# dongzhuoyao/self-guided-diffusion-models

Measured on AMD Instinct MI355X. Metric: cfg_sampled_images_per_sec_64x64_1000step_ddpm, higher is better.
Workload: dtype f32 as 3xf16 split MFMA products, f32 accumulate; 1 GPU; IN64 unet_fast ch128 cluster-k5000 cond_scale=2 bs=40/GPU (UNet batch 80), 1000-step native DDPM; batch_per_gpu=40, unet_batch=80, precision_mode=f16x3, launch=hipGraph-captured step

## Files before the change

include/sgdm_hip.h:

```cpp
#ifndef SGDM_HIP_H
#define SGDM_HIP_H
#include <stdint.h>

#ifdef __cplusplus
extern "C" {
#endif

#define SGD_ABI_VERSION 24
int sgd_abi_version(void);
const char* sgd_build_id(void);

enum { SGD_MODE_FLAT = 0, SGD_MODE_CONV3 = 1 };
enum { SGD_RS_NONE = 0, SGD_RS_AVGPOOL2 = 1, SGD_RS_UP2 = 2,
       SGD_RS_ZEROUP2 = 3 ,
       SGD_RS_UP2_SUBPIXEL = 4 };
enum { SGD_PRO_NONE = 0, SGD_PRO_AFFINE_NC = 1, SGD_PRO_LN_ROW = 2 };
enum { SGD_PREC_F32 = 0, SGD_PREC_F16X3 = 1, SGD_PREC_BF16X3 = 2, SGD_PREC_F16 = 3, SGD_PREC_BF16 = 4 };

typedef struct sgd_igemm_args {
    const float* x0;
    const float* x1;
    int32_t c0, c1;
    int32_t mode;
    int32_t n, hi, wi;
    int32_t ho, wo;
    int32_t m;
    int32_t rows_per_n;
    int32_t stride;
    int32_t resample;
    int32_t pro;
    int32_t pro_silu;
    const float* pa;
    const float* pb;
    const float* pc;
    const void* w;
    int32_t cin_p, cout_p;
    const float* bias;
    const float* res;
    int32_t res_mode;
    float* y;
    int32_t cout;
    int32_t y_ld;
    int32_t orows_in, orows_out, orow_off;
    int32_t prec;
    float drop_p;
    uint32_t drop_seed;
    float* stats;
    const float* w_scale_inv;
    void* work;
    int64_t work_bytes;
    int32_t grid_cap;
    int32_t tune;
} sgd_igemm_args;
enum {
    SGD_TUNE_BN128 = 1,
    SGD_TUNE_BN256 = 2,
    SGD_TUNE_FLAT2 = 4,
    SGD_TUNE_DEFER = 8,
    SGD_TUNE_PLAIN_SCHEDULE = 16,
    SGD_TUNE_NO_SMALL = 64,
    SGD_TUNE_LN_PACKED = 32,
    SGD_TUNE_WGRAD_GENERIC_NARROW = 256,
// ... 38 lines not shown
    float* scale_inv;
    int32_t cout, cin, ksize, transpose;
    int32_t own_amax, reserved0;
} sgd_pack_job;
int sgd_pack_job_blocks(int32_t cout, int32_t cin, int32_t ksize, int32_t prec, int32_t transpose, int32_t* amax_blocks,
                        int32_t* pack_blocks, int32_t* cin_p, int32_t* cout_p );
int sgd_pack_weights_batched(const sgd_pack_job* jobs, int32_t n_jobs, const int32_t* amax_block_job, const int32_t* amax_first,
                             int32_t n_amax_blocks, const int32_t* pack_block_job, const int32_t* pack_first,
                             int32_t n_pack_blocks, int32_t prec, void* stream);

int sgd_linear_splitk(const float* x, int32_t x_ld, const float* w, const float* bias, int32_t m, int32_t n, int32_t k,
                      float* work, int32_t ksplit, float* y, int32_t y_ld, void* stream);
int sgd_linear_splitk_t(const float* x, int32_t x_ld, const float* w, int32_t w_ld, int32_t m, int32_t n, int32_t k,
                        float* work, int32_t ksplit, float* y, int32_t y_ld, void* stream);

int sgd_chan_stats(const float* x, int32_t n, int32_t hw, int32_t c,
                   float* sums , int32_t c_total, int32_t c_off, void* stream);
int sgd_add_rows_nc(float* x, const float* e, int32_t e_ld, int32_t n, int64_t hw, int32_t c, void* stream);
int sgd_stats_reduce(const float* partial, int32_t n, int32_t parts, int32_t c,
                     float* sums , int32_t c_total, int32_t c_off, void* stream);
int sgd_gn_coef_parts(const float* partial0, int32_t parts0, int32_t c0, const float* partial1, int32_t parts1, int32_t c1,
                      float* sums, const float* gamma, const float* beta, const float* film, int32_t film_ld,
                      int32_t n, int32_t groups, int32_t hw, float eps, float* a, float* b, void* stream);
int sgd_gn_coef(const float* sums, const float* gamma, const float* beta,
                const float* film , int32_t film_ld,
                int32_t n, int32_t c, int32_t groups, int32_t hw, float eps,
                float* a, float* b, void* stream);

int sgd_ln_stats(const float* x, int32_t rows, int32_t c, float eps, float* stats , void* stream);
int sgd_ln_apply(const float* x, const float* gamma, const float* beta, const float* res,
                 int32_t rows, int32_t c, float eps, float* out, void* stream);

int sgd_attention(const float* q, int32_t q_ld, int32_t q_hs,
                  const float* k, const float* v, int32_t kv_ld, int32_t kv_hs,
                  int32_t batch, int32_t heads, int32_t tq, int32_t tk, int32_t d, float scale,
                  float* out, int32_t out_ld,
                  float* lse ,
                  void* stream);
int sgd_attention_split(const float* q, int32_t q_ld, int32_t q_hs,
                        const float* k, const float* v, int32_t kv_ld, int32_t kv_hs,
                        int32_t batch, int32_t heads, int32_t tq, int32_t tk, int32_t d, float scale,
                        float* out, int32_t out_ld, float* lse, void* stream);

int sgd_timestep_embedding(const int64_t* t, const float* freqs, int32_t n_src, int32_t n, int32_t dim,
                           float* out, void* stream);
int sgd_cond_select(const void* cond, int32_t is_i64, const uint8_t* mask, const float* null_row,
// ... 170 lines not shown
```

self-guided-diffusion-models_amd/csrc/backward.hip:

```cpp
#include "sgdm_common.h"
#include "../../include/sgdm_hip.h"
#include "prologue.h"

namespace {

__device__ __forceinline__ float dsilu(float z) {
    const float s = 1.0f / (1.0f + __expf(-z));
    return s * (1.0f + z * (1.0f - s));
}

constexpr int WK = 64;
constexpr int WT = 128;
constexpr int WLD = WT + 4;

struct WArgs {
    sgd_igemm_args a;
    const float* gy;
    int gy_ld, cout, ksplit, taps, rows, co_tiles, ci_tiles, ktiles, hc, wc, wo_l2, ho_l2, gvec;
    float* slabs;
    float* bslab;
    const void* gh; const void* gl; const void* uh; const void* ul;
    int no_flat_pipe;
    int tap9;
};
// ... 1611 lines not shown
static bool wgrad_ws_ok(const sgd_igemm_args& a, int cout, int gy_ld) {
    const bool vec = (a.c0 % 4 == 0) && (a.c1 % 4 == 0);
    const bool pooled = a.resample == SGD_RS_AVGPOOL2 && !(a.tune & SGD_TUNE_WGRAD_NO_POOLED_PLANES);
    return wgrad_fast_conv(a) && a.prec != SGD_PREC_F32 && !(a.tune & SGD_TUNE_WGRAD_F32) && vec && gy_ld % 4 == 0 && cout % WT == 0
           && (a.resample == SGD_RS_NONE || a.resample == SGD_RS_UP2 || pooled)
           && (a.pro == SGD_PRO_NONE || a.pro == SGD_PRO_AFFINE_NC) && !(a.tune & SGD_TUNE_WGRAD_NO_WS);
}
static int64_t wgrad_planes_need(const sgd_igemm_args& a, int cout) {
    const int64_t rows = (int64_t)a.n * a.ho * a.wo;
    return 4 * (rows * cout + (int64_t)a.n * a.hi * a.wi * (a.c0 + a.c1));
}
static bool wgrad_planes_ok(const sgd_igemm_args& a, int cout, int gy_ld, bool have_scratch, int64_t scratch_bytes) {
    if (!(wgrad_ws_ok(a, cout, gy_ld) && have_scratch && scratch_bytes >= wgrad_planes_need(a, cout) && !(a.tune & SGD_TUNE_WGRAD_NO_PLANES)))
        return false;
    const long cin = a.c0 + a.c1;
    return cin * cout > 100 * (cin + cout) || a.resample == SGD_RS_AVGPOOL2 || (a.tune & SGD_TUNE_WGRAD_PLANES_ALWAYS);
}

static int wgrad_impl(const sgd_igemm_args* fwd, const float* gy, int32_t gy_ld, int32_t cout, float* slabs,
                      int32_t ksplit, float* bias_slabs, void* scratch, int64_t scratch_bytes, void* stream) {
    SGD_CLEAR_ERR();
    if (!fwd || !gy || !slabs || cout <= 0 || ksplit <= 0 || gy_ld < cout) return SGD_ERR_ARG;
    if (fwd->prec < SGD_PREC_F32 || fwd->prec > SGD_PREC_BF16X3) return SGD_ERR_ARG;
    WArgs w;
    w.a = *fwd;
    w.no_flat_pipe = (fwd->tune & SGD_TUNE_WGRAD_NO_PIPE) ? 1 : 0;
    w.tap9 = 0;
    const sgd_igemm_args& a = w.a;
    if (!a.x0 || a.c0 <= 0 || a.c1 < 0 || (a.c1 > 0 && !a.x1)) return SGD_ERR_ARG;
    if (a.pro != SGD_PRO_NONE && (!a.pa || !a.pb)) return SGD_ERR_ARG;
    const int cin = a.c0 + a.c1;
    if (a.mode == SGD_MODE_CONV3) {
        if (a.stride != 1 && a.stride != 2) return SGD_ERR_ARG;
        w.hc = a.resample == SGD_RS_AVGPOOL2 ? a.hi / 2 : (a.resample == SGD_RS_UP2 ? a.hi * 2 : a.hi);
        w.wc = a.resample == SGD_RS_AVGPOOL2 ? a.wi / 2 : (a.resample == SGD_RS_UP2 ? a.wi * 2 : a.wi);
        w.taps = 9;
        w.rows = a.n * a.ho * a.wo;
        if (a.ho <= 0 || a.wo <= 0 || (a.ho & (a.ho - 1)) || (a.wo & (a.wo - 1))) return SGD_ERR_ARG;
        w.wo_l2 = __builtin_ctz(a.wo);
        w.ho_l2 = __builtin_ctz(a.ho);
    } else if (a.mode == SGD_MODE_FLAT) {
        w.hc = w.wc = 1;
        w.wo_l2 = w.ho_l2 = 0;
        w.taps = 1;
        w.rows = a.m;
    } else {
// ... 271 lines not shown
```

self-guided-diffusion-models_amd/csrc/igemm.hip:

```cpp
#include <type_traits>
#include <utility>

#include "igemm_shared.h"
#include "prologue.h"

namespace {

#ifdef SGDM_PROBE
#define DBG(bit) 0
#define SYNC() do { if (g.stamp) { const unsigned long long t0_ = __builtin_amdgcn_s_memtime(); __syncthreads(); \
                    const unsigned long long t1_ = __builtin_amdgcn_s_memtime(); \
                    if (g.trace && blockIdx.x < 16 && pr_nbar < 512 && (threadIdx.x & 63) == 0) { \
                        unsigned long long* tp_ = g.trace + (((size_t)blockIdx.x * (NTHREADS / 64) + (threadIdx.x >> 6)) * 512 + pr_nbar) * 2; \
                        tp_[0] = t0_; tp_[1] = t1_; } \
                    pr_bar += t1_ - t0_; ++pr_nbar; } else if (!DBG(64)) { __syncthreads(); } } while (0)
#define PROBE_BEGIN() unsigned long long pr_bar = 0, pr_nbar = 0, pr_epi = 0; const unsigned long long pr_t0 = __builtin_amdgcn_s_memtime()
#define PROBE_END(role) do { if (g.stamp && (threadIdx.x & 63) == 0) { \
        unsigned long long* sp_ = g.stamp + ((size_t)blockIdx.x * (NTHREADS / 64) + (threadIdx.x >> 6)) * 4; \
        sp_[0] = __builtin_amdgcn_s_memtime() - pr_t0; sp_[1] = pr_bar; sp_[2] = pr_nbar; sp_[3] = pr_epi; } } while (0)
#define PROBE_EPI(expr) do { if (g.stamp) { const unsigned long long t0_ = __builtin_amdgcn_s_memtime(); expr; pr_epi += __builtin_amdgcn_s_memtime() - t0_; } else { expr; } } while (0)
#else
#define DBG(bit) 0
#define SYNC() __syncthreads()
#define PROBE_BEGIN()
// ... 318 lines not shown

        Q = (ntiles - 1) * nchunks + (last_c1 - last_c0);
        S = Q * TAPS;
        s = CONV ? a.stride : 1;
        TW = 1 << g.tw_l2; TH = 1 << g.th_l2;
        M = CONV ? a.n * a.ho * a.wo : a.m;

        return true;
    }

    __device__ __forceinline__ void build_pixtab(int k, int t0, int nthr) const {
        if (k >= ntiles) return;
        const Tile T = tile_at<SUBPIX>(g, lin_of(k), BN, TW, TH);
        int2* tab = pixtab + (size_t)(k & 3) * g.pix;
        for (int pix = t0; pix < g.pix; pix += nthr) {
            int2 e;
            e.x = -1;
            e.y = 0;
            if (CONV) {
                int hx = pix % g.hw, t = pix / g.hw;
                int hy = t % g.hh, nb = t / g.hh;
                int n = T.img0 + nb, y = T.ty0 * s - 1 + hy, x = T.tx0 * s - 1 + hx;
                if (n < a.n && y >= 0 && y < g.hc && x >= 0 && x < g.wc) {
                    if (a.resample == SGD_RS_UP2) e.x = (n * a.hi + (y >> 1)) * a.wi + (x >> 1);
                    else if (a.resample == SGD_RS_AVGPOOL2) e.x = (n * a.hi + 2 * y) * a.wi + 2 * x;
                    else if (a.resample == SGD_RS_ZEROUP2) e.x = ((y | x) & 1) ? -1 : (n * a.hi + (y >> 1)) * a.wi + (x >> 1);
                    else e.x = (n * a.hi + y) * a.wi + x;
                    e.y = n;
                }
            } else {
                long row = T.m0 + pix;
                if (row < M) {
                    e.x = (int)row;
                    e.y = (a.pro == SGD_PRO_AFFINE_NC) ? (int)(row / a.rows_per_n) : 0;
                }
            }
            tab[pix] = e;
        }
    }

    static constexpr size_t SLAB = (size_t)RB * CBN * QPB * NCOMP * 16;
    static __device__ __forceinline__ f32x4 accq(const AccV (&acc)[RB][CBN], int mt, int nt, int q) {
        f32x4 v;
#pragma unroll
        for (int j = 0; j < 4; ++j) v[j] = acc[mt][nt][(M16 ? 0 : q * 4) + j];
        return v;
    }
    __device__ __forceinline__ int pixel_of_lane(int ln) const {
    const int l5 = ln & 31;
        int px = l5;
// ... 1104 lines not shown
```

self-guided-diffusion-models_amd/csrc/igemm_host.hip:

```cpp
#include <stdint.h>

#include "igemm_shared.h"

extern "C" int sgd_abi_version(void) { return SGD_ABI_VERSION; }

static inline int pick_bn(int cout) { return (cout % 128 == 0) ? 128 : 32; }

static inline int column_tile(const sgd_igemm_args& a) {
    const int bn = pick_bn(a.cout);
    if (bn != 128 || (a.tune & (SGD_TUNE_NO_SMALL | SGD_TUNE_BN128 | SGD_TUNE_BN256))) return bn;
    const long rows = a.mode == SGD_MODE_CONV3 ? (long)a.n * a.ho * a.wo : (long)a.m;
    const long t128 = ((rows + BM - 1) / BM) * ((a.cout + 127) / 128);
    return t128 * 4 <= device_cus() ? 32 : 128;
}

static int make_geo(const sgd_igemm_args& a, Geo& g, int bn, int& na, int fg = 1) {
    if (a.c0 <= 0 || a.c1 < 0 || a.cout <= 0 || a.y_ld < a.cout) return SGD_ERR_ARG;
    if (a.mode == SGD_MODE_CONV3) {
        if (a.n <= 0 || a.hi <= 0 || a.wi <= 0 || (a.stride != 1 && a.stride != 2)) return SGD_ERR_ARG;
        if (a.stride == 2 && a.resample != SGD_RS_NONE) return SGD_ERR_ARG;
        if (a.resample < SGD_RS_NONE || a.resample > SGD_RS_UP2_SUBPIXEL) return SGD_ERR_ARG;
        const bool sub = a.resample == SGD_RS_UP2_SUBPIXEL;
        const bool up = a.resample == SGD_RS_UP2 || a.resample == SGD_RS_ZEROUP2;
        g.hc = a.resample == SGD_RS_AVGPOOL2 ? a.hi / 2 : (up ? a.hi * 2 : a.hi);
// ... 105 lines not shown
    Geo g;
    int na;
    if (make_geo(a, g, 128, na) != SGD_OK) return false;
    if (a.stats && g.sparts == 0) return false;
    const size_t smem = (size_t)na * g.pix * LDA * sizeof(float) + (size_t)g.pix * 32
                        + (a.cout <= BIAS_LDS_MAX ? (size_t)((a.cout + 127) / 128 * 128) * sizeof(float) : 0);
    return smem <= 160 * 1024;
}

extern "C" int sgd_igemm_subpixel_ok(const sgd_igemm_args* args) { return args && subpixel_ok(*args) ? 1 : 0; }

extern "C" int sgd_igemm(const sgd_igemm_args* args, void* stream) {
    SGD_CLEAR_ERR();
    if (!args) return SGD_ERR_ARG;
    KArgs ka;
    ka.a = *args;
    sgd_igemm_args& a = ka.a;
    Geo& g = ka.g;
    if (!a.x0 || !a.w || !a.y || a.c0 <= 0 || a.c1 < 0 || a.cout <= 0) return SGD_ERR_ARG;
    if (a.prec < SGD_PREC_F32 || a.prec > SGD_PREC_BF16) return SGD_ERR_ARG;
    if (a.c1 > 0 && (!a.x1 || a.c0 % KC != 0)) return SGD_ERR_ARG;
    if (a.y_ld < a.cout) return SGD_ERR_ARG;
    if (a.pro != SGD_PRO_NONE && (!a.pa || !a.pb)) return SGD_ERR_ARG;
    const int cin = a.c0 + a.c1;
    int bn = column_tile(a);
    if (a.cout_p % pick_bn(a.cout) != 0 || a.cout_p < a.cout || a.cin_p % KC != 0 || a.cin_p < cin) return SGD_ERR_ARG;
    const bool vec = (a.c0 % 4 == 0) && (a.c1 % 4 == 0);
    const bool conv = a.mode == SGD_MODE_CONV3;
    const bool sub = conv && a.resample == SGD_RS_UP2_SUBPIXEL;
    if (sub && !subpixel_ok(a)) return SGD_ERR_ARG;
    if (bn == 128 && a.cout_p % 256 == 0 && vec && (!a.res || a.res_mode == SGD_RS_NONE) && want_bn256(a)) bn = 256;
    int na;
    int taps = conv ? (sub ? 4 : 9) : 1;
    const bool ln_nopk = !conv && a.pro == SGD_PRO_LN_ROW && a.prec != SGD_PREC_F32 && !(a.tune & SGD_TUNE_LN_PACKED);
    const bool ln_any = !conv && a.pro == SGD_PRO_LN_ROW && (ln_nopk || (a.tune & SGD_TUNE_LN_PACKED));
    if (!conv && vec && bn >= 128 && a.drop_p == 0.f && cin % (2 * KC) == 0 && (a.c1 == 0 || a.c0 % KC == 0)
        && (a.pro == SGD_PRO_NONE || (a.pro == SGD_PRO_AFFINE_NC && a.rows_per_n > 0 && a.rows_per_n % BM == 0) || ln_any)
        && (a.tune & SGD_TUNE_FLAT2))
        taps = 2;
    {
        const int rc = make_geo(a, g, bn, na, conv ? 1 : taps);
        if (rc != SGD_OK) return rc;
    }
    if (a.stats && g.sparts == 0) return SGD_ERR_ARG;
    g.nt = a.cout_p / bn;
    if ((a.work && a.work_bytes < sgd_igemm_work_bytes()) || (a.tune & SGD_TUNE_PLAIN_SCHEDULE)) a.work = nullptr;
// ... 47 lines not shown
```

self-guided-diffusion-models_amd/csrc/norm.hip:

```cpp
#include "sgdm_common.h"
#include "../../include/sgdm_hip.h"

namespace {

__global__ __launch_bounds__(256) void chan_stats_kernel(const float* __restrict__ x, int hw, int c,
                                                         float* __restrict__ sums, int c_total, int c_off) {
    const int slabs = (c + 31) / 32;
    const int n = blockIdx.x / slabs, slab = blockIdx.x % slabs;
    const int q = threadIdx.x & 7, rl = threadIdx.x >> 3;
    const int ch = slab * 32 + q * 4;
    float s[4] = {0, 0, 0, 0}, ss[4] = {0, 0, 0, 0};
    const float* base = x + (long)n * hw * c;
    if (ch < c) {
        if ((c & 3) == 0) {
            for (int r = rl; r < hw; r += 32) {
                f32x4 v = *reinterpret_cast<const f32x4*>(base + (long)r * c + ch);
#pragma unroll
                for (int j = 0; j < 4; ++j) { s[j] += v[j]; ss[j] += v[j] * v[j]; }
            }
        } else {
            for (int r = rl; r < hw; r += 32)
#pragma unroll
                for (int j = 0; j < 4; ++j)
                    if (ch + j < c) { float v = base[(long)r * c + ch + j]; s[j] += v; ss[j] += v * v; }
// ... 46 lines not shown
    for (int k = 0; k < cpg; ++k) {
        s += sums[((long)nn * c + g0 + k) * 2];
        ss += sums[((long)nn * c + g0 + k) * 2 + 1];
    }
    const double cnt = (double)cpg * hw;
    const double mean = s / cnt;
    double var = ss / cnt - mean * mean;
    if (var < 0) var = 0;
    const double rstd = 1.0 / sqrt(var + (double)eps);
    double ga = gamma[cc] * rstd, be = beta[cc] - mean * ga;
    if (film) {
        const double sc = 1.0 + film[(long)nn * film_ld + cc], sh = film[(long)nn * film_ld + c + cc];
        ga *= sc;
        be = be * sc + sh;
    }
    a[i] = (float)ga;
    b[i] = (float)be;
}

__global__ __launch_bounds__(512) void gn_coef_parts_kernel(const float* __restrict__ p0, int parts0, int c0,
                                                            const float* __restrict__ p1, int parts1, int c1,
                                                            float* __restrict__ sums, const float* __restrict__ gamma,
                                                            const float* __restrict__ beta, const float* __restrict__ film,
                                                            int film_ld, int groups, int hw, float eps,
                                                            float* __restrict__ a, float* __restrict__ b) {
    extern __shared__ double shd[];
    const int nn = blockIdx.x, c = c0 + c1, nthr = blockDim.x;
    const int G = c < nthr ? nthr / c : 1;
    float* sh = reinterpret_cast<float*>(shd + (size_t)G * c * 2);
    for (int it = threadIdx.x; it < c * G; it += nthr) {
        const int ch = it % c, grp = it / c;
        const bool first = ch < c0;
        const float* p = first ? p0 : p1;
        const int parts = first ? parts0 : parts1, cs = first ? c0 : c1, cl = first ? ch : ch - c0;
        double t0 = 0, t1 = 0;
        if (parts > 0) {
            const float* q = p + (long)nn * parts * 2 * cs + cl;
            int k = grp;
            for (; k + 7 * G < parts; k += 8 * G) {
                float v0[8], v1[8];
#pragma unroll
                for (int j = 0; j < 8; ++j) { v0[j] = q[(long)(k + j * G) * 2 * cs]; v1[j] = q[(long)(k + j * G) * 2 * cs + cs]; }
#pragma unroll
                for (int j = 0; j < 8; ++j) { t0 += v0[j]; t1 += v1[j]; }
            }
            if (k + 3 * G < parts) {
                float v0[4], v1[4];
#pragma unroll
                for (int j = 0; j < 4; ++j) { v0[j] = q[(long)(k + j * G) * 2 * cs]; v1[j] = q[(long)(k + j * G) * 2 * cs + cs]; }
#pragma unroll
                for (int j = 0; j < 4; ++j) { t0 += v0[j]; t1 += v1[j]; }
                k += 4 * G;
            }
            for (; k < parts; k += G) { t0 += q[(long)k * 2 * cs]; t1 += q[(long)k * 2 * cs + cs]; }
        }
        shd[((size_t)grp * c + ch) * 2] = t0;
        shd[((size_t)grp * c + ch) * 2 + 1] = t1;
    }
    __syncthreads();
    for (int ch = threadIdx.x; ch < c; ch += nthr) {
// ... 164 lines not shown

extern "C" int sgd_stats_reduce(const float* partial, int32_t n, int32_t parts, int32_t c, float* sums,
                                int32_t c_total, int32_t c_off, void* stream) {
    SGD_CLEAR_ERR();
    if (!partial || !sums || n <= 0 || parts <= 0 || c <= 0 || c_off < 0 || c_off + c > c_total) return SGD_ERR_ARG;
    hipLaunchKernelGGL(stats_reduce_kernel, dim3((2 * c + 31) / 32, n), dim3(256), 0, (hipStream_t)stream, partial,
                       parts, c, sums, c_total, c_off);
    return sgd_check_launch();
}

extern "C" int sgd_gn_coef(const float* sums, const float* gamma, const float* beta, const float* film,
                           int32_t film_ld, int32_t n, int32_t c, int32_t groups, int32_t hw, float eps, float* a,
                           float* b, void* stream) {
    SGD_CLEAR_ERR();
    if (!sums || !gamma || !beta || !a || !b || n <= 0 || c <= 0 || groups <= 0 || c % groups != 0 || hw <= 0)
        return SGD_ERR_ARG;
    if (film && film_ld < 2 * c) return SGD_ERR_ARG;
    const long total = (long)n * c;
    hipLaunchKernelGGL(gn_coef_kernel, dim3((unsigned)((total + 255) / 256)), dim3(256), 0, (hipStream_t)stream,
                       sums, gamma, beta, film, film_ld, n, c, groups, hw, eps, a, b);
    return sgd_check_launch();
}

extern "C" int sgd_gn_coef_parts(const float* p0, int32_t parts0, int32_t c0, const float* p1, int32_t parts1, int32_t c1,
                                 float* sums, const float* gamma, const float* beta, const float* film, int32_t film_ld,
                                 int32_t n, int32_t groups, int32_t hw, float eps, float* a, float* b, void* stream) {
    SGD_CLEAR_ERR();
    const int c = c0 + c1;
    if (!sums || !gamma || !beta || !a || !b || n <= 0 || c0 <= 0 || c1 < 0 || groups <= 0 || c % groups != 0 || hw <= 0 ||
        parts0 < 0 || parts1 < 0 || (parts0 > 0 && !p0) || (c1 > 0 && parts1 > 0 && !p1) || c > 8192)
        return SGD_ERR_ARG;
    if (film && film_ld < 2 * c) return SGD_ERR_ARG;
    const int nthr = 512, G = c < nthr ? nthr / c : 1;
    const size_t lds = (size_t)G * c * 2 * sizeof(double) + (size_t)c * 2 * sizeof(float);
    if (lds > 160 * 1024) return SGD_ERR_ARG;
    if (lds > 64 * 1024) {
        static bool raised = false;
        if (!raised) {
            (void)hipFuncSetAttribute((const void*)gn_coef_parts_kernel, hipFuncAttributeMaxDynamicSharedMemorySize, 160 * 1024);
            raised = true;
        }
    }
    hipLaunchKernelGGL(gn_coef_parts_kernel, dim3(n), dim3(nthr), lds,
                       (hipStream_t)stream, p0, parts0, c0, p1, parts1, c1, sums, gamma, beta, film, film_ld, groups, hw, eps, a, b);
    return sgd_check_launch();
}

extern "C" int sgd_ln_stats(const float* x, int32_t rows, int32_t c, float eps, float* stats, void* stream) {
    SGD_CLEAR_ERR();
    if (!x || !stats || rows <= 0 || c <= 0 || c > 1024) return SGD_ERR_ARG;
    hipLaunchKernelGGL((ln_kernel<false>), dim3((rows + 3) / 4), dim3(256), 0, (hipStream_t)stream, x,
                       (const float*)nullptr, (const float*)nullptr, (const float*)nullptr, rows, c, eps, stats);
    return sgd_check_launch();
}

extern "C" int sgd_ln_apply(const float* x, const float* gamma, const float* beta, const float* res, int32_t rows,
                            int32_t c, float eps, float* out, void* stream) {
    SGD_CLEAR_ERR();
    if (!x || !gamma || !out || rows <= 0 || c <= 0 || c > 1024) return SGD_ERR_ARG;
    hipLaunchKernelGGL((ln_kernel<true>), dim3((rows + 3) / 4), dim3(256), 0, (hipStream_t)stream, x, gamma, beta,
                       res, rows, c, eps, out);
    return sgd_check_launch();
}

extern "C" int sgd_ln_bwd(const float* x, const float* g, const float* gamma, int32_t rows, int32_t c, float eps,
                          float* dst, int32_t accumulate, float* gxhat, const float* gres, void* stream) {
    SGD_CLEAR_ERR();
    if (!x || !g || !gamma || !dst || rows <= 0 || c <= 0 || c > 1024) return SGD_ERR_ARG;
// ... 5 lines not shown
```

self-guided-diffusion-models_amd/sgdm_amd/_lib.py:

```python
import ctypes as C
import os

import torch

_HERE = os.path.dirname(os.path.abspath(__file__))
LIB_PATH = os.environ.get("SGDM_LIB_PATH") or os.path.join(_HERE, "lib", "libsgdm_hip.so")

MODE_FLAT, MODE_CONV3 = 0, 1
RS_NONE, RS_AVGPOOL2, RS_UP2, RS_ZEROUP2, RS_UP2_SUBPIXEL = 0, 1, 2, 3, 4
PRO_NONE, PRO_AFFINE_NC, PRO_LN_ROW = 0, 1, 2
PREC_F32, PREC_F16X3, PREC_BF16X3, PREC_F16, PREC_BF16 = 0, 1, 2, 3, 4
PREC_BY_NAME = {"f32": PREC_F32, "f16x3": PREC_F16X3, "bf16x3": PREC_BF16X3, "f16": PREC_F16, "bf16": PREC_BF16}
INFERENCE_ONLY = ("f16", "bf16")
ABI_VERSION = 24

TUNE_BN128, TUNE_BN256, TUNE_FLAT2, TUNE_DEFER, TUNE_PLAIN_SCHEDULE, TUNE_LN_PACKED, TUNE_NO_SMALL = 1, 2, 4, 8, 16, 32, 64
TUNE_WGRAD_GENERIC_NARROW, TUNE_WGRAD_NO_POOLED_PLANES, TUNE_WGRAD_F32 = 256, 512, 1024
TUNE_WGRAD_NO_WS, TUNE_WGRAD_NO_PLANES, TUNE_WGRAD_NO_PIPE, TUNE_WGRAD_PLANES_ALWAYS = 2048, 4096, 8192, 16384
TUNE_NO_SUBPIXEL = 32768
PACK_FORWARD, PACK_DGRAD, PACK_SUBPIXEL = 0, 1, 2

vp, i32, i64, f32 = C.c_void_p, C.c_int32, C.c_int64, C.c_float


class IgemmArgs(C.Structure):
    _fields_ = [
        ("x0", vp), ("x1", vp), ("c0", i32), ("c1", i32), ("mode", i32),
        ("n", i32), ("hi", i32), ("wi", i32), ("ho", i32), ("wo", i32), ("m", i32),
        ("rows_per_n", i32), ("stride", i32), ("resample", i32), ("pro", i32), ("pro_silu", i32),
        ("pa", vp), ("pb", vp), ("pc", vp), ("w", vp), ("cin_p", i32), ("cout_p", i32),
        ("bias", vp), ("res", vp), ("res_mode", i32), ("y", vp), ("cout", i32), ("y_ld", i32),
        ("orows_in", i32), ("orows_out", i32), ("orow_off", i32), ("prec", i32),
        ("drop_p", f32), ("drop_seed", C.c_uint32), ("stats", vp), ("w_scale_inv", vp),
        ("work", vp), ("work_bytes", i64), ("grid_cap", i32), ("tune", i32),
    ]


class PackJob(C.Structure):
    _fields_ = [("src", vp), ("dst", vp), ("amax_bits", vp), ("scale_inv", vp), ("cout", i32), ("cin", i32), ("ksize", i32),
                ("transpose", i32), ("own_amax", i32), ("reserved0", i32)]


SIGNATURES = {
    "sgd_abi_version": (i32, []),
    "sgd_build_id": (C.c_char_p, []),
    "sgd_igemm": (i32, [C.POINTER(IgemmArgs), vp]),
    "sgd_igemm_stats_parts": (i32, [C.POINTER(IgemmArgs)]),
    "sgd_igemm_subpixel_ok": (i32, [C.POINTER(IgemmArgs)]),
    "sgd_igemm_work_bytes": (i64, []),
    "sgd_igemm_work_status_offset": (i64, []),
    "sgd_igemm_tail_layout": (i32, [i32, i32, i32, i32, C.POINTER(i32)]),
    "sgd_stats_reduce": (i32, [vp, i32, i32, i32, vp, i32, i32, vp]),
    "sgd_packed_weight_bytes": (i64, [i32, i32, i32, i32]),
    "sgd_pack_weight": (i32, [vp, vp, i32, i32, i32, i32, C.POINTER(i32), C.POINTER(i32), vp]),
    "sgd_weight_amax": (i32, [vp, i64, vp, vp]),
    "sgd_pack_weight_scaled": (i32, [vp, vp, i32, i32, i32, i32, i32, vp, vp, C.POINTER(i32), C.POINTER(i32), vp]),
    "sgd_packed_weight_subpixel_bytes": (i64, [i32, i32, i32]),
    "sgd_weight_amax_subpixel": (i32, [vp, i32, i32, vp, vp]),
    "sgd_pack_weight_subpixel_scaled": (i32, [vp, vp, i32, i32, i32, vp, vp, C.POINTER(i32), C.POINTER(i32), vp]),
    "sgd_pack_job_blocks": (i32, [i32, i32, i32, i32, i32, C.POINTER(i32), C.POINTER(i32), C.POINTER(i32), C.POINTER(i32)]),
    "sgd_pack_weights_batched": (i32, [vp, i32, vp, vp, i32, vp, vp, i32, i32, vp]),
    "sgd_linear_splitk": (i32, [vp, i32, vp, vp, i32, i32, i32, vp, i32, vp, i32, vp]),
    "sgd_linear_splitk_t": (i32, [vp, i32, vp, i32, i32, i32, i32, vp, i32, vp, i32, vp]),
    "sgd_conv3_narrow_in_parts": (i32, [i32, i32]),
    "sgd_conv3_narrow_in": (i32, [vp, vp, vp, vp, vp, i32, i32, i32, i32, i32, i32, i32, vp]),
    "sgd_conv3_narrow_out": (i32, [vp, vp, vp, i32, vp, vp, vp, i32, i32, i32, i32, i32, i32, vp]),
    "sgd_chan_stats": (i32, [vp, i32, i32, i32, vp, i32, i32, vp]),
    "sgd_gn_coef_parts": (i32, [vp, i32, i32, vp, i32, i32, vp, vp, vp, vp, i32, i32, i32, i32, f32, vp, vp, vp]),
    "sgd_gn_coef": (i32, [vp, vp, vp, vp, i32, i32, i32, i32, i32, f32, vp, vp, vp]),
    "sgd_add_rows_nc": (i32, [vp, vp, i32, i32, i64, i32, vp]),
    "sgd_ln_stats": (i32, [vp, i32, i32, f32, vp, vp]),
    "sgd_ln_apply": (i32, [vp, vp, vp, vp, i32, i32, f32, vp, vp]),
    "sgd_attention": (i32, [vp, i32, i32, vp, vp, i32, i32, i32, i32, i32, i32, i32, f32, vp, i32, vp, vp]),
    "sgd_attention_split": (i32, [vp, i32, i32, vp, vp, i32, i32, i32, i32, i32, i32, i32, f32, vp, i32, vp, vp]),
    "sgd_attention_masked": (i32, [vp, i32, i32, vp, vp, i32, i32, vp, i32, i32, i32, i32, i32, f32, vp, i32, vp, vp]),
    "sgd_linear_attention": (i32, [vp, i32, i32, vp, vp, i32, i32, vp, i32, i32, i32, i32, i32, f32, vp, i32, vp]),
    "sgd_attention_bwd": (i32, [vp, i32, i32, vp, vp, i32, i32, vp, i32, vp, i32, vp, vp, i32, i32, i32, i32, i32, f32,
                              vp, vp, vp, vp]),
    "sgd_attention_bwd_split": (i32, [vp, i32, i32, vp, vp, i32, i32, vp, i32, vp, i32, vp, vp, i32, i32, i32, i32, i32, f32,
                                    vp, vp, vp, vp]),
    "sgd_attention_masked_bwd": (i32, [vp, i32, i32, vp, vp, i32, i32, vp, vp, i32, vp, i32, vp, vp, i32, i32, i32, i32, i32,
                                     f32, vp, vp, vp, vp]),
    "sgd_linear_attention_bwd": (i32, [vp, i32, i32, vp, vp, i32, i32, vp, vp, i32, i32, i32, i32, i32, i32, f32, vp, vp, vp,
                                     vp]),
    "sgd_pack_weight_dgrad": (i32, [vp, vp, i32, i32, i32, i32, C.POINTER(i32), C.POINTER(i32), vp]),
    "sgd_wgrad": (i32, [C.POINTER(IgemmArgs), vp, i32, i32, vp, i32, vp, vp]),
    "sgd_wgrad_scratch_bytes": (i64, [C.POINTER(IgemmArgs), i32]),
    "sgd_wgrad_scratch": (i32, [C.POINTER(IgemmArgs), vp, i32, i32, vp, i32, vp, vp, i64, vp]),
    "sgd_colsum_fold": (i32, [vp, i32, i32, vp, i32, f32, vp]),
    "sgd_wgrad_reduce": (i32, [vp, i32, i32, i32, i32, vp, i32, f32, vp]),
    "sgd_wgrad_reduce_bias": (i32, [vp, i32, i32, i32, i32, vp, i32, f32, vp, i32, vp, vp]),
# ... 104 lines not shown
```

self-guided-diffusion-models_amd/sgdm_amd/unet.py:

```python
import ctypes as C
import weakref
import math
import os

import torch
import torch.nn as nn

from . import _lib as L

GN_GROUPS, GN_EPS, LN_EPS = 32, 1e-5, 1e-5
NUM_TIME_TOKENS = NUM_COND_TOKENS = 8


def _ptr(t):
    return C.c_void_p(t.data_ptr()) if t is not None else C.c_void_p(0)


def timestep_freqs(dim, max_period=10000):
    half = dim // 2
    return torch.exp(-math.log(max_period) * torch.arange(start=0, end=half, dtype=torch.float32) / half)


def default_precision():
    return os.environ.get("SGDM_PREC", "f32")
# ... 487 lines not shown


def grad_health(dev):
    dev = torch.device(dev)
    key = (dev.type, dev.index if dev.index is not None else (torch.cuda.current_device() if dev.type == "cuda" else 0))
    if key not in _GRAD_HEALTH:
        _GRAD_HEALTH[key] = torch.zeros(1, dtype=torch.float32, device=dev)
    return _GRAD_HEALTH[key]


class _Engine:

    def __init__(self, model, n, h, w, prec, dev):
        self.m, self.n, self.h, self.w, self.prec, self.dev = model, n, h, w, prec, dev
        self.lib = L.load()
        self.prog = _Program()
        self.packed = []
        self.bufs = []
        self.tape = []
        self.drops = []
        self.lse = {}
        self.stats_of = {}
        self._p_drop = 0.0
        self._grid_cap = 0
        self.refresh_hooks = []
        self.work_bytes = int(self.lib.sgd_igemm_work_bytes()) if os.environ.get("SGDM_BALANCE", "1") != "0" else 0
        self.work = torch.zeros(max(1, self.work_bytes // 4), dtype=torch.float32, device=dev)
        self._build()

    def buf(self, *shape, dtype=torch.float32):
        t = torch.empty(*shape, dtype=dtype, device=self.dev)
        self.bufs.append(t)
        return t

    def attention_fn(self):
        return self.lib.sgd_attention_split if self.prec in (L.PREC_F16X3, L.PREC_F16) else self.lib.sgd_attention

    def pack(self, names, ksize, pad=None, subpixel=False):
        pk = _Packed([self.m.P(nm) for nm in names], ksize, self.prec, pad, subpixel)
        self.packed.append(pk)
        return pk

    def up_conv(self, tag, x0, c0, y, cout, wname, conv, *, stats=False, **kw):
        assert conv[6] == L.RS_UP2
        pk = self.pack([wname], 3)
        q = L.IgemmArgs()
# ... 98 lines not shown
                return fn(x_p, pa_p, pb_p, int(silu), w_p, b_p, y_p, nimg, ho, wo, c0, cout, y_ld, stream)
            self.prog.add(tag, sgd_conv3_narrow_out, flops=flops, nbytes=nbytes)
        elif launch:
            self.prog.add(tag, self.lib.sgd_igemm, C.byref(a), flops=flops, nbytes=nbytes)
        return a

    def gn(self, tag, srcs, hw, gname, film=None, film_ld=0, eps=GN_EPS):
        n = self.n
        ct = sum(c for _, c in srcs)
        sums = self.buf(n, ct, 2)
        off = 0
        parts = []
        for t, c in srcs:
            st = self.stats_of.get(t.data_ptr())
            if st is not None and st[2] == c:
                parts.append((st[0], st[1], c))
            else:
                self.prog.add(tag + ".stats", self.lib.sgd_chan_stats, _ptr(t), n, hw, c, _ptr(sums), ct, off)
                parts.append((None, 0, c))
            off += c
        a, b = self.buf(n, ct), self.buf(n, ct)
        self._last_sums = sums
        gw, gb = self.m.P(gname + ".weight"), self.m.P(gname + ".bias")
        if len(parts) <= 2 and any(p[1] > 0 for p in parts):
            (p0, n0, c0), (p1, n1, c1) = parts[0], (parts[1] if len(parts) == 2 else (None, 0, 0))
            self.prog.add(tag + ".coef", self.lib.sgd_gn_coef_parts, _ptr(p0) if p0 is not None else None, n0, c0,
                          _ptr(p1) if p1 is not None else None, n1, c1, _ptr(sums), _ptr(gw), _ptr(gb),
                          C.c_void_p(film or 0), film_ld, n, GN_GROUPS, hw, eps, _ptr(a), _ptr(b))
        else:
            self.prog.add(tag + ".coef", self.lib.sgd_gn_coef, _ptr(sums), _ptr(gw), _ptr(gb), C.c_void_p(film or 0),
                          film_ld, n, ct, GN_GROUPS, hw, eps, _ptr(a), _ptr(b))
        return a, b

    def _build(self):
        m, n, H, W = self.m, self.n, self.h, self.w
        self._late = []
        mc = m.model_channels
        ted = 4 * mc
        P = m.P
        lib = self.lib
        self.temb = self.buf(n, mc)
        self.freqs = timestep_freqs(mc).to(self.dev)
        cin_tot = m._in_ch_total
        self.x_in = self.buf(n, H, W, cin_tot)
        self.cond_m = self.buf(n, max(1, m._cond_width)) if m._cond_width else None
        emb = self.buf(n, ted)
        e1 = self.buf(n, ted)
        a0 = self.igemm("time_embed.0", self.temb, mc, e1, ted, self.pack(["time_embed.0.weight"], 1), m=n,
                        bias=P("time_embed.0.bias"))
        a2 = self.igemm("time_embed.2", e1, ted, emb, ted, self.pack(["time_embed.2.weight"], 1), m=n, silu=1,
                        bias=P("time_embed.2.bias"))
        self.tape.append(dict(kind="mlp2", name="time_embed", x=self.temb, h=e1, y=emb, a0=a0, a2=a2, cin=mc,
                              mid=ted, cout=ted, add_to_y=False))
        self.context = None
        self.emb_c = None
# ... 57 lines not shown
                               stats=True)
                self.tape.append(dict(kind="down", p=p, x=t, y=y, c=c, hw_in=(hh, ww), a=a))
                srcs = [(y, c, hh // 2, ww // 2)]
            elif kind == "up":
                (t, c, hh, ww), = srcs
                y = self.buf(self.n, hh * 2, ww * 2, c)
                a = self.up_conv(p + ".conv", t, c, y, c, p + ".conv.weight",
                                 (self.n, hh, ww, hh * 2, ww * 2, 1, L.RS_UP2), bias=self.m.P(p + ".conv.bias"), stats=True)
                self.tape.append(dict(kind="up", p=p, x=t, y=y, c=c, hw_in=(hh, ww), a=a))
                srcs = [(y, c, hh * 2, ww * 2)]
        return srcs[0]

    def _res(self, p, layer, srcs):
        _, cin, cout, ud = layer
        n, P = self.n, self.m.P
        t0, c0, hh, ww = srcs[0]
        t1, c1 = (srcs[1][0], srcs[1][1]) if len(srcs) == 2 else (None, 0)
        assert c0 + c1 == cin
        rs = {None: L.RS_NONE, "down": L.RS_AVGPOOL2, "up": L.RS_UP2}[ud]
        ho, wo = (hh // 2, ww // 2) if ud == "down" else ((hh * 2, ww * 2) if ud == "up" else (hh, ww))
        ss = self.m.use_scale_shift_norm
        a1, b1 = self.gn(p + ".in_layers.0", [(t0, c0)] + ([(t1, c1)] if t1 is not None else []), hh * ww,
                         p + ".in_layers.0")
        sums1 = self._last_sums
        h1 = self.buf(n, ho, wo, cout)
        kw1 = dict(x1=t1, c1=c1, pro=L.PRO_AFFINE_NC, silu=1, pa=a1, pb=b1, bias=P(p + ".in_layers.2.bias"), stats=ss)
        if rs == L.RS_UP2:
            ac1 = self.up_conv(p + ".in_layers.2", t0, c0, h1, cout, p + ".in_layers.2.weight", (n, hh, ww, ho, wo, 1, rs), **kw1)
        else:
            ac1 = self.igemm(p + ".in_layers.2", t0, c0, h1, cout, self.pack([p + ".in_layers.2.weight"], 3),
                             conv=(n, hh, ww, ho, wo, 1, rs), **kw1)
        film_ptr = self.film.data_ptr() + 4 * self.film_off[p]
        if ss:
            a2, b2 = self.gn(p + ".out_layers.0", [(h1, cout)], ho * wo, p + ".out_layers.0", film=film_ptr,
                             film_ld=self.film_ld)
        else:
            self.prog.add(p + ".emb_add", self.lib.sgd_add_rows_nc, _ptr(h1), C.c_void_p(film_ptr), self.film_ld, n, ho * wo, cout)
            a2, b2 = self.gn(p + ".out_layers.0", [(h1, cout)], ho * wo, p + ".out_layers.0")
        sums2 = self._last_sums
        ask = None
        if cin != cout:
            assert ud is None
            skip = self.buf(n, hh, ww, cout)
            ask = self.igemm(p + ".skip_connection", t0, c0, skip, cout,
                             self.pack([p + ".skip_connection.weight"], 1), x1=t1, c1=c1, m=n * hh * ww,
                             bias=P(p + ".skip_connection.bias"))
            res, res_mode = skip, L.RS_NONE
        else:
            assert t1 is None
            res, res_mode = t0, rs
        y = self.buf(n, ho, wo, cout)
        ac2 = self.igemm(p + ".out_layers.3", h1, cout, y, cout, self.pack([p + ".out_layers.3.weight"], 3),
                         conv=(n, ho, wo, ho, wo, 1, L.RS_NONE), pro=L.PRO_AFFINE_NC, silu=1, pa=a2, pb=b2,
                         bias=P(p + ".out_layers.3.bias"), res=res, res_mode=res_mode, stats=True)
        pbox, sbox = C.c_float(0.0), C.c_uint32(0)
        self.drops.append((ac2, pbox, sbox))
        self.tape.append(dict(kind="res", drop_p=pbox, drop_seed=sbox, p=p,
                              srcs=[(t0, c0)] + ([(t1, c1)] if t1 is not None else []), cin=cin,
                              cout=cout, hw_in=(hh, ww), hw_out=(ho, wo), rs=rs, a1=a1, b1=b1, sums1=sums1, h1=h1,
                              a2=a2, b2=b2, sums2=sums2, film_off=self.film_off[p], conv1=ac1, conv2=ac2, skip=ask,
                              y=y, ss=ss))
        return (y, cout, ho, wo)

    def refresh(self, stream):
        if getattr(self, "_pack_batch", None) is None or len(self._pack_batch.packs) != len(self.packed):
            self._pack_batch = _PackBatch(self.packed, self.prec, self.dev)
        self._pack_batch.refresh(stream)
        for a, pk in self._late:
            a.cin_p, a.cout_p = pk.cin_p, pk.cout_p
        for hook in self.refresh_hooks:
            hook(stream)
        sig = tuple((b.data_ptr(), b._version) for b in self._film_bias_src)
        if sig != getattr(self, "_film_sig", None):
            self._film_bias.copy_(torch.cat([b.detach().reshape(-1) for b in self._film_bias_src]))
            self._film_sig = sig

    def _health_fail(self, training=False):
        self.work.zero_()
        what = ("sgdm_amd: a conv launch's balanced tail timed out waiting for another block's partial sums (stale arrival "
# ... 47 lines not shown
            bw.apply_grid_cap()

    def run(self, x, t, cond, layout, mask, train=False):
        stream = torch.cuda.current_stream().cuda_stream
        self.prepare(x, t, cond, layout, mask, train=train)
        self.launch(stream)

    def prepare(self, x, t, cond, layout, mask, train=False):
        m, n = self.m, self.n
        stream = torch.cuda.current_stream().cuda_stream
        self.poll_health()
        self.refresh(stream)
        from .ddp import reserved_cus
        self.set_grid_cap(reserved_cus(m) if train else 0)
        p_drop = float(m.dropout) if (train and m.dropout) else 0.0
        if p_drop != self._p_drop or p_drop > 0:
            seeds = torch.randint(0, 2 ** 31 - 1, (len(self.drops),)).tolist() if p_drop > 0 else [0] * len(self.drops)
            for (a, pbox, sbox), sd in zip(self.drops, seeds):
                a.drop_p, a.drop_seed = p_drop, sd
                pbox.value, sbox.value = p_drop, sd
            self._p_drop = p_drop
        B = x.shape[0]
        assert n % B == 0
        x = x.contiguous().float()
        t = t.contiguous().to(torch.int64)
        mask_u8 = mask.contiguous().view(torch.uint8) if mask is not None else None
        cl = m._in_ch_total - m.in_channels
        lfmt = 0
        if cl:
            if layout is None:
                raise ValueError(f"condition_method={m.condition_method} needs `layout`")
            if layout.dtype == torch.uint8 and layout.numel() == B * self.h * self.w:
                layout, lfmt = layout.contiguous(), 1
            elif layout.dtype in (torch.int32, torch.int64) and tuple(layout.shape) == (B, 4):
                if cl != 1:
                    raise ValueError("box-corner layouts need layout_dim == 1")
                layout, lfmt = layout.to(torch.int32).contiguous(), 2
            else:
                layout = layout.contiguous().float()
                assert layout.shape == (B, cl, self.h, self.w), (layout.shape, (B, cl, self.h, self.w))
        is_i64 = 0
        if m._cond_width:
            if cond is None:
                raise ValueError(f"condition_method={m.condition_method} needs `cond`")
            cond = cond.contiguous()
            if cond.dtype == torch.int64 and cond.numel() == B and m._cond_width > 1:
# ... 532 lines not shown
```

Baseline: 2.325 images/s.

## Share first resblock conv and GN stats between CFG cond/uncond halves

```diff
diff --git a/include/sgdm_hip.h b/include/sgdm_hip.h
--- a/include/sgdm_hip.h
+++ b/include/sgdm_hip.h
@@ -38,6 +38,7 @@
     const float* bias;
     const float* res;
     int32_t res_mode;
+    int32_t x_imgs;
     float* y;
     int32_t cout;
     int32_t y_ld;
@@ -122,6 +123,9 @@
 int sgd_gn_coef_parts(const float* partial0, int32_t parts0, int32_t c0, const float* partial1, int32_t parts1, int32_t c1,
                       float* sums, const float* gamma, const float* beta, const float* film, int32_t film_ld,
                       int32_t n, int32_t groups, int32_t hw, float eps, float* a, float* b, void* stream);
+int sgd_gn_coef_parts_shared(const float* partial0, int32_t parts0, int32_t c0, const float* partial1, int32_t parts1, int32_t c1,
+                             float* sums, const float* gamma, const float* beta, const float* film, int32_t film_ld,
+                             int32_t n, int32_t stats_imgs, int32_t groups, int32_t hw, float eps, float* a, float* b, void* stream);
 int sgd_gn_coef(const float* sums, const float* gamma, const float* beta,
                 const float* film , int32_t film_ld,
                 int32_t n, int32_t c, int32_t groups, int32_t hw, float eps,
diff --git a/self-guided-diffusion-models_amd/csrc/backward.hip b/self-guided-diffusion-models_amd/csrc/backward.hip
--- a/self-guided-diffusion-models_amd/csrc/backward.hip
+++ b/self-guided-diffusion-models_amd/csrc/backward.hip
@@ -1657,6 +1657,7 @@
     SGD_CLEAR_ERR();
     if (!fwd || !gy || !slabs || cout <= 0 || ksplit <= 0 || gy_ld < cout) return SGD_ERR_ARG;
     if (fwd->prec < SGD_PREC_F32 || fwd->prec > SGD_PREC_BF16X3) return SGD_ERR_ARG;
+    if (fwd->x_imgs != 0) return SGD_ERR_ARG;
     WArgs w;
     w.a = *fwd;
     w.no_flat_pipe = (fwd->tune & SGD_TUNE_WGRAD_NO_PIPE) ? 1 : 0;
diff --git a/self-guided-diffusion-models_amd/csrc/igemm.hip b/self-guided-diffusion-models_amd/csrc/igemm.hip
--- a/self-guided-diffusion-models_amd/csrc/igemm.hip
+++ b/self-guided-diffusion-models_amd/csrc/igemm.hip
@@ -364,10 +364,11 @@
                 int hy = t % g.hh, nb = t / g.hh;
                 int n = T.img0 + nb, y = T.ty0 * s - 1 + hy, x = T.tx0 * s - 1 + hx;
                 if (n < a.n && y >= 0 && y < g.hc && x >= 0 && x < g.wc) {
-                    if (a.resample == SGD_RS_UP2) e.x = (n * a.hi + (y >> 1)) * a.wi + (x >> 1);
-                    else if (a.resample == SGD_RS_AVGPOOL2) e.x = (n * a.hi + 2 * y) * a.wi + 2 * x;
-                    else if (a.resample == SGD_RS_ZEROUP2) e.x = ((y | x) & 1) ? -1 : (n * a.hi + (y >> 1)) * a.wi + (x >> 1);
-                    else e.x = (n * a.hi + y) * a.wi + x;
+                    const int ns = a.x_imgs > 0 ? n % a.x_imgs : n;
+                    if (a.resample == SGD_RS_UP2) e.x = (ns * a.hi + (y >> 1)) * a.wi + (x >> 1);
+                    else if (a.resample == SGD_RS_AVGPOOL2) e.x = (ns * a.hi + 2 * y) * a.wi + 2 * x;
+                    else if (a.resample == SGD_RS_ZEROUP2) e.x = ((y | x) & 1) ? -1 : (ns * a.hi + (y >> 1)) * a.wi + (x >> 1);
+                    else e.x = (ns * a.hi + y) * a.wi + x;
                     e.y = n;
                 }
             } else {
diff --git a/self-guided-diffusion-models_amd/csrc/igemm_host.hip b/self-guided-diffusion-models_amd/csrc/igemm_host.hip
--- a/self-guided-diffusion-models_amd/csrc/igemm_host.hip
+++ b/self-guided-diffusion-models_amd/csrc/igemm_host.hip
@@ -151,6 +151,7 @@
     if (a.c1 > 0 && (!a.x1 || a.c0 % KC != 0)) return SGD_ERR_ARG;
     if (a.y_ld < a.cout) return SGD_ERR_ARG;
     if (a.pro != SGD_PRO_NONE && (!a.pa || !a.pb)) return SGD_ERR_ARG;
+    if (a.x_imgs < 0 || (a.x_imgs > 0 && (a.mode != SGD_MODE_CONV3 || a.drop_p != 0.f))) return SGD_ERR_ARG;
     const int cin = a.c0 + a.c1;
     int bn = column_tile(a);
     if (a.cout_p % pick_bn(a.cout) != 0 || a.cout_p < a.cout || a.cin_p % KC != 0 || a.cin_p < cin) return SGD_ERR_ARG;
diff --git a/self-guided-diffusion-models_amd/csrc/norm.hip b/self-guided-diffusion-models_amd/csrc/norm.hip
--- a/self-guided-diffusion-models_amd/csrc/norm.hip
+++ b/self-guided-diffusion-models_amd/csrc/norm.hip
@@ -92,10 +92,11 @@
                                                             const float* __restrict__ p1, int parts1, int c1,
                                                             float* __restrict__ sums, const float* __restrict__ gamma,
                                                             const float* __restrict__ beta, const float* __restrict__ film,
-                                                            int film_ld, int groups, int hw, float eps,
+                                                            int film_ld, int stats_imgs, int groups, int hw, float eps,
                                                             float* __restrict__ a, float* __restrict__ b) {
     extern __shared__ double shd[];
     const int nn = blockIdx.x, c = c0 + c1, nthr = blockDim.x;
+    const int ns = stats_imgs > 0 ? nn % stats_imgs : nn;
     const int G = c < nthr ? nthr / c : 1;
     float* sh = reinterpret_cast<float*>(shd + (size_t)G * c * 2);
     for (int it = threadIdx.x; it < c * G; it += nthr) {
@@ -105,7 +106,7 @@
         const int parts = first ? parts0 : parts1, cs = first ? c0 : c1, cl = first ? ch : ch - c0;
         double t0 = 0, t1 = 0;
         if (parts > 0) {
-            const float* q = p + (long)nn * parts * 2 * cs + cl;
+            const float* q = p + (long)ns * parts * 2 * cs + cl;
             int k = grp;
             for (; k + 7 * G < parts; k += 8 * G) {
                 float v0[8], v1[8];
@@ -316,11 +317,13 @@
     return sgd_check_launch();
 }
 
-extern "C" int sgd_gn_coef_parts(const float* p0, int32_t parts0, int32_t c0, const float* p1, int32_t parts1, int32_t c1,
-                                 float* sums, const float* gamma, const float* beta, const float* film, int32_t film_ld,
-                                 int32_t n, int32_t groups, int32_t hw, float eps, float* a, float* b, void* stream) {
+extern "C" int sgd_gn_coef_parts_shared(const float* p0, int32_t parts0, int32_t c0, const float* p1, int32_t parts1, int32_t c1,
+                                        float* sums, const float* gamma, const float* beta, const float* film, int32_t film_ld,
+                                        int32_t n, int32_t stats_imgs, int32_t groups, int32_t hw, float eps, float* a, float* b,
+                                        void* stream) {
     SGD_CLEAR_ERR();
     const int c = c0 + c1;
+    if (stats_imgs < 0) return SGD_ERR_ARG;
     if (!sums || !gamma || !beta || !a || !b || n <= 0 || c0 <= 0 || c1 < 0 || groups <= 0 || c % groups != 0 || hw <= 0 ||
         parts0 < 0 || parts1 < 0 || (parts0 > 0 && !p0) || (c1 > 0 && parts1 > 0 && !p1) || c > 8192)
         return SGD_ERR_ARG;
@@ -336,8 +339,14 @@
         }
     }
     hipLaunchKernelGGL(gn_coef_parts_kernel, dim3(n), dim3(nthr), lds,
-                       (hipStream_t)stream, p0, parts0, c0, p1, parts1, c1, sums, gamma, beta, film, film_ld, groups, hw, eps, a, b);
-    return sgd_check_launch();
+                       (hipStream_t)stream, p0, parts0, c0, p1, parts1, c1, sums, gamma, beta, film, film_ld, stats_imgs, groups, hw, eps, a, b);
+    return sgd_check_launch();
+}
+
+extern "C" int sgd_gn_coef_parts(const float* p0, int32_t parts0, int32_t c0, const float* p1, int32_t parts1, int32_t c1,
+                                 float* sums, const float* gamma, const float* beta, const float* film, int32_t film_ld,
+                                 int32_t n, int32_t groups, int32_t hw, float eps, float* a, float* b, void* stream) {
+    return sgd_gn_coef_parts_shared(p0, parts0, c0, p1, parts1, c1, sums, gamma, beta, film, film_ld, n, 0, groups, hw, eps, a, b, stream);
 }
 
 extern "C" int sgd_ln_stats(const float* x, int32_t rows, int32_t c, float eps, float* stats, void* stream) {
diff --git a/self-guided-diffusion-models_amd/sgdm_amd/_lib.py b/self-guided-diffusion-models_amd/sgdm_amd/_lib.py
--- a/self-guided-diffusion-models_amd/sgdm_amd/_lib.py
+++ b/self-guided-diffusion-models_amd/sgdm_amd/_lib.py
@@ -29,7 +29,7 @@
         ("n", i32), ("hi", i32), ("wi", i32), ("ho", i32), ("wo", i32), ("m", i32),
         ("rows_per_n", i32), ("stride", i32), ("resample", i32), ("pro", i32), ("pro_silu", i32),
         ("pa", vp), ("pb", vp), ("pc", vp), ("w", vp), ("cin_p", i32), ("cout_p", i32),
-        ("bias", vp), ("res", vp), ("res_mode", i32), ("y", vp), ("cout", i32), ("y_ld", i32),
+        ("bias", vp), ("res", vp), ("res_mode", i32), ("x_imgs", i32), ("y", vp), ("cout", i32), ("y_ld", i32),
         ("orows_in", i32), ("orows_out", i32), ("orow_off", i32), ("prec", i32),
         ("drop_p", f32), ("drop_seed", C.c_uint32), ("stats", vp), ("w_scale_inv", vp),
         ("work", vp), ("work_bytes", i64), ("grid_cap", i32), ("tune", i32),
@@ -67,6 +67,7 @@
     "sgd_conv3_narrow_out": (i32, [vp, vp, vp, i32, vp, vp, vp, i32, i32, i32, i32, i32, i32, vp]),
     "sgd_chan_stats": (i32, [vp, i32, i32, i32, vp, i32, i32, vp]),
     "sgd_gn_coef_parts": (i32, [vp, i32, i32, vp, i32, i32, vp, vp, vp, vp, i32, i32, i32, i32, f32, vp, vp, vp]),
+    "sgd_gn_coef_parts_shared": (i32, [vp, i32, i32, vp, i32, i32, vp, vp, vp, vp, i32, i32, i32, i32, i32, f32, vp, vp, vp]),
     "sgd_gn_coef": (i32, [vp, vp, vp, vp, i32, i32, i32, i32, i32, f32, vp, vp, vp]),
     "sgd_add_rows_nc": (i32, [vp, vp, i32, i32, i64, i32, vp]),
     "sgd_ln_stats": (i32, [vp, i32, i32, f32, vp, vp]),
diff --git a/self-guided-diffusion-models_amd/sgdm_amd/unet.py b/self-guided-diffusion-models_amd/sgdm_amd/unet.py
--- a/self-guided-diffusion-models_amd/sgdm_amd/unet.py
+++ b/self-guided-diffusion-models_amd/sgdm_amd/unet.py
@@ -533,6 +533,8 @@
         self.lse = {}
         self.stats_of = {}
         self._p_drop = 0.0
+        self._prefix = None
+        self._prefix_imgs = 0
         self._grid_cap = 0
         self.refresh_hooks = []
         self.work_bytes = int(self.lib.sgd_igemm_work_bytes()) if os.environ.get("SGDM_BALANCE", "1") != "0" else 0
@@ -677,6 +679,7 @@
         a, b = self.buf(n, ct), self.buf(n, ct)
         self._last_sums = sums
         gw, gb = self.m.P(gname + ".weight"), self.m.P(gname + ".bias")
+        self._last_coef_op = len(self.prog.ops) if len(parts) == 1 and parts[0][1] > 0 else None
         if len(parts) <= 2 and any(p[1] > 0 for p in parts):
             (p0, n0, c0), (p1, n1, c1) = parts[0], (parts[1] if len(parts) == 2 else (None, 0, 0))
             self.prog.add(tag + ".coef", self.lib.sgd_gn_coef_parts, _ptr(p0) if p0 is not None else None, n0, c0,
@@ -686,6 +689,39 @@
             self.prog.add(tag + ".coef", self.lib.sgd_gn_coef, _ptr(sums), _ptr(gw), _ptr(gb), C.c_void_p(film or 0),
                           film_ld, n, ct, GN_GROUPS, hw, eps, _ptr(a), _ptr(b))
         return a, b
+
+    def _note_prefix(self, coef1, conv1_op, conv1, coef2, h1, cout):
+        if (self.m._in_ch_total != self.m.in_channels or coef1 is None or coef2 is None or not conv1.stats or self.n < 2
+                or len(self.prog.ops) < conv1_op + 2 or self.prog.ops[conv1_op][1] is not self.lib.sgd_igemm):
+            return
+        q = L.IgemmArgs.from_buffer_copy(conv1)
+        q.n = 1
+        parts_max = self.lib.sgd_igemm_stats_parts(C.byref(q))
+        if parts_max <= 0:
+            return
+        self._prefix = dict(coef1=coef1, conv1=conv1, coef2=coef2, h1=h1, conv2=None, stats_full=conv1.stats,
+                            stats=self.buf(self.n // 2, parts_max, 2, cout), parts_max=parts_max,
+                            full={i: self.prog.ops[i] for i in (coef1, coef2)})
+
+    def _share_prefix(self, imgs):
+        px = self._prefix
+        if px is None or px["conv2"] is None or imgs == self._prefix_imgs:
+            return
+        n, c1, c2 = self.n, px["conv1"], px["conv2"]
+        for i, op in px["full"].items():
+            self.prog.ops[i] = op
+        c1.n, c1.stats, c2.x_imgs = n, px["stats_full"], 0
+        if imgs:
+            c1.n, c1.stats = imgs, px["stats"].data_ptr()
+            parts = self.lib.sgd_igemm_stats_parts(C.byref(c1))
+            assert 0 < parts <= px["parts_max"], (parts, px["parts_max"])
+            c2.x_imgs = imgs
+            name, fn, a = px["full"][px["coef1"]]
+            self.prog.ops[px["coef1"]] = (name, fn, a[:11] + (imgs,) + a[12:])
+            name, fn, a = px["full"][px["coef2"]]
+            self.prog.ops[px["coef2"]] = (name, self.lib.sgd_gn_coef_parts_shared,
+                                          (_ptr(px["stats"]), parts) + a[2:12] + (imgs,) + a[12:])
+        self._prefix_imgs = imgs
 
     def _build(self):
         m, n, H, W = self.m, self.n, self.h, self.w
@@ -789,8 +825,9 @@
         ss = self.m.use_scale_shift_norm
         a1, b1 = self.gn(p + ".in_layers.0", [(t0, c0)] + ([(t1, c1)] if t1 is not None else []), hh * ww,
                          p + ".in_layers.0")
-        sums1 = self._last_sums
+        sums1, coef1 = self._last_sums, self._last_coef_op
         h1 = self.buf(n, ho, wo, cout)
+        conv1_op = len(self.prog.ops)
         kw1 = dict(x1=t1, c1=c1, pro=L.PRO_AFFINE_NC, silu=1, pa=a1, pb=b1, bias=P(p + ".in_layers.2.bias"), stats=ss)
         if rs == L.RS_UP2:
             ac1 = self.up_conv(p + ".in_layers.2", t0, c0, h1, cout, p + ".in_layers.2.weight", (n, hh, ww, ho, wo, 1, rs), **kw1)
@@ -801,6 +838,8 @@
         if ss:
             a2, b2 = self.gn(p + ".out_layers.0", [(h1, cout)], ho * wo, p + ".out_layers.0", film=film_ptr,
                              film_ld=self.film_ld)
+            if p == "input_blocks.1.0" and rs == L.RS_NONE and t1 is None:
+                self._note_prefix(coef1, conv1_op, ac1, self._last_coef_op, h1, cout)
         else:
             self.prog.add(p + ".emb_add", self.lib.sgd_add_rows_nc, _ptr(h1), C.c_void_p(film_ptr), self.film_ld, n, ho * wo, cout)
             a2, b2 = self.gn(p + ".out_layers.0", [(h1, cout)], ho * wo, p + ".out_layers.0")
@@ -822,6 +861,8 @@
                          bias=P(p + ".out_layers.3.bias"), res=res, res_mode=res_mode, stats=True)
         pbox, sbox = C.c_float(0.0), C.c_uint32(0)
         self.drops.append((ac2, pbox, sbox))
+        if self._prefix is not None and self._prefix["h1"] is h1:
+            self._prefix["conv2"] = ac2
         self.tape.append(dict(kind="res", drop_p=pbox, drop_seed=sbox, p=p,
                               srcs=[(t0, c0)] + ([(t1, c1)] if t1 is not None else []), cin=cin,
                               cout=cout, hw_in=(hh, ww), hw_out=(ho, wo), rs=rs, a1=a1, b1=b1, sums1=sums1, h1=h1,
@@ -915,6 +956,7 @@
             self._p_drop = p_drop
         B = x.shape[0]
         assert n % B == 0
+        self._share_prefix(B if B < n and not train and os.environ.get("SGDM_CFG_SHARE", "1") != "0" else 0)
         x = x.contiguous().float()
         t = t.contiguous().to(torch.int64)
         mask_u8 = mask.contiguous().view(torch.uint8) if mask is not None else None
```

Measured after the change: 2.336 images/s (median of 6 runs). About the same (+0.5%).
